# philipturner/metal-flash-attention

Hardware: NVIDIA H100
Metric: giga-FMA-instr/sec forward attn N=4096 D=128 bf16 (higher is better)
Workload: dtype bf16

## Files before the change

### metal-flash-attention_b200/csrc/kernel.cpp

```cpp
#include <cuda_runtime.h>

#include <algorithm>
#include <cmath>
#include <cstring>
#include <map>
#include <mutex>
#include <string>
#include <vector>

#include "internal.h"
#include "kernels/device_state.h"

struct mfa_attention_kernel {
  mfa_attention_kernel_descriptor_t descriptor;
  int type;
  int backend;
  uint32_t threads, smem_bytes, par, trav, head;
  std::string source_name;
  bool windowed;
  mfa_attention_window_t window;
};

namespace mfa {

// ... 245 lines not shown
    if (!precision_pair_valid(mem, reg)) return fail(MFA_ERROR_INVALID_PRECISIONS, "Invalid precisions.");
    if (op != MFA_L && op != MFA_D && !((kd->transpose_state_valid_mask >> op) & 1))
      return fail(MFA_ERROR_INCOMPLETE_DESCRIPTOR,
                  std::string("Transpose state of ") + mfa_operand_name((mfa_operand_t)op) + " was not specified.");
  }

  mfa_attention_kernel *k = new mfa_attention_kernel();
  k->descriptor = *kd;
  k->type = kd->type;
  k->backend = kd->backend;
  const uint32_t D = kd->head_dimension;

  if (k->backend == MFA_BACKEND_TCGEN05) {
    const uint8_t pq = kd->memory_precisions[MFA_Q];
    const uint32_t Dp = (D + 7) / 8 * 8;
    bool ok = (pq == MFA_FP16 || pq == MFA_BF16) && kd->memory_precisions[MFA_K] == pq &&
              kd->memory_precisions[MFA_V] == pq && Dp <= kWgmmaMaxHead;
    bool transposed = false;
    for (int i = 0; i < n; ++i)
      if ((kd->transpose_state_mask >> ops[i]) & 1) transposed = true;
    if (transposed && D % 8 != 0) ok = false;
    if (k->type != MFA_FORWARD && kd->memory_precisions[MFA_dO] != pq &&
        !(pq == MFA_FP16 && kd->memory_precisions[MFA_dO] == MFA_BF16))
      ok = false;
    if (!ok) {
      delete k;
      return fail(MFA_ERROR_UNSUPPORTED,
                  "MFA_BACKEND_TCGEN05 needs FP16/BF16 Q,K,V (row-major for head % 8 != 0; dO of the same "
                  "type, or BF16 with FP16 Q,K,V) and pad8(head) <= the compiled maximum; use MFA_BACKEND_SIMT_FP32 for this "
                  "descriptor.");
    }
    const WgmmaPlan plan = wgmma_plan(k->type, Dp, 1, 1, 1, 1, 0, 1, false, 1);
    k->threads = plan.threads;
    k->smem_bytes = plan.smem_bytes;
    k->par = plan.par;
    k->trav = plan.trav;
    k->head = plan.head;
  } else if (k->backend == MFA_BACKEND_SIMT_FP32) {
    if (D > 512) {
      delete k;
      return fail(MFA_ERROR_UNSUPPORTED, "Head dimension " + std::to_string(D) + " exceeds 512.");
    }
    simt_geometry(k->type, D, &k->threads, &k->smem_bytes, &k->par, &k->trav, &k->head);
  } else {
    delete k;
    return fail(MFA_ERROR_INVALID_ARGUMENT, "Unrecognized backend.");
  }
  if (kd->block_parallelization != k->par || kd->block_traversal != k->trav) {
    std::string msg = "Block dimensions " + std::to_string(kd->block_parallelization) + "x" +
                      std::to_string(kd->block_traversal) + " have no compiled sm_90a kernel (available: " +
                      std::to_string(k->par) + "x" + std::to_string(k->trav) + ").";
    delete k;
    return fail(MFA_ERROR_UNSUPPORTED, msg);
  }
  static const char *typeNames[] = {"forward", "backward_query", "backward_key_value"};
  k->source_name = std::string("attention_") + typeNames[k->type] +
                   (k->backend == MFA_BACKEND_TCGEN05 ? "_tcgen05" : "_simt_fp32") + "<D=" + std::to_string(D) +
                   ">" + (kd->causal ? "_causal" : "");
  k->windowed = false;
  k->window = mfa_attention_window_t{-1, -1};
  *out = k;
  return MFA_SUCCESS;
}

int mfa_attention_kernel_create_windowed(const mfa_attention_kernel_descriptor_t *kd, const mfa_attention_window_t *window,
                                         mfa_attention_kernel_t **out) {
  if (!kd || !out) return fail(MFA_ERROR_INVALID_ARGUMENT, "NULL argument.");
// ... 618 lines not shown
```

### metal-flash-attention_b200/csrc/kernels/attention_params.h

```cpp
#pragma once
#include <cuda_runtime.h>
#include <stdint.h>

namespace mfa {

enum Slot { sQ = 0, sK = 1, sV = 2, sO = 3, sL = 4, sD = 5, sdO = 6, sdV = 7, sdK = 8, sdQ = 9, kSlots = 10 };

enum Prec : uint8_t { FP32 = 0, FP16 = 1, BF16 = 2 };

struct AttentionParams {
  uint32_t R;
  uint32_t C;
  uint32_t D;
  uint32_t batch;
  uint32_t group;
  void *buf[kSlots];
  uint8_t prec[kSlots];
  uint8_t transposed[kSlots];
  float scale;
  float scale_log2;
  uint8_t split_min_blocks;
  uint8_t split_max;
  uint8_t causal;
  int32_t causal_offset;
// ... 52 lines not shown

cudaError_t launch_simt_forward(const AttentionParams &p, const Sequences *seq, const Band *band, cudaStream_t stream);
cudaError_t launch_simt_backward_query(const AttentionParams &p, const Sequences *seq, const Band *band,
                                       cudaStream_t stream);
cudaError_t launch_simt_backward_key_value(const AttentionParams &p, const Sequences *seq, const Band *band,
                                           cudaStream_t stream);
cudaError_t launch_simt_forward_paged(const AttentionParams &p, const PagedKV &pk, const Band *band,
                                      cudaStream_t stream);
void simt_geometry(int type, uint32_t D, uint32_t *threads, uint32_t *smem_bytes, uint32_t *par, uint32_t *trav,
                   uint32_t *head);

constexpr uint32_t kWgmmaMaxHead = 256;
cudaError_t launch_wgmma_forward(const AttentionParams &p, const Sequences *seq, const Band *band, cudaStream_t stream);
cudaError_t launch_wgmma_backward_query(const AttentionParams &p, const Sequences *seq, const Band *band,
                                        cudaStream_t stream);
cudaError_t launch_wgmma_backward_key_value(const AttentionParams &p, const Sequences *seq, const Band *band,
                                            cudaStream_t stream);
cudaError_t launch_wgmma_forward_paged(const AttentionParams &p, const PagedKV &pk, const Band *band,
                                       cudaStream_t stream);
cudaError_t launch_wgmma_forward_split(const AttentionParams &p, const Sequences *seq, const PagedKV *pk,
                                       const Band *band, uint32_t num_splits, uint32_t key_bound, cudaStream_t stream);

struct WgmmaPlan {
  uint32_t threads, smem_bytes;
  uint32_t par, trav, head;
  dim3 grid;
  uint32_t blocks_per_split, splits;
  bool convert_dO_first;
  uint32_t launches;
  uint32_t heads_per_tile;
};
WgmmaPlan wgmma_plan(int type, uint32_t D, uint32_t R, uint32_t C, uint32_t batch, uint32_t group, uint32_t min_blocks,
                     uint32_t max_splits, bool convert_dO, uint32_t sm_count, const Band *band = nullptr);
WgmmaPlan wgmma_plan_sequences(int type, uint32_t D, uint32_t max_row, uint32_t max_column, uint32_t count,
                               uint32_t batch, uint32_t group, bool convert_dO, uint32_t sm_count);
WgmmaPlan wgmma_plan_split(uint32_t D, uint32_t max_row, uint32_t key_bound, uint32_t count, uint32_t batch,
                           uint32_t group, uint32_t min_blocks, uint32_t max_splits, uint32_t num_splits,
                           uint32_t sm_count, const Band *band);

cudaError_t launch_stage_operand(const void *src, void *dst, uint32_t batch, uint32_t seq, uint32_t D, uint32_t Dp,
                                 uint32_t element_bytes, bool transposed, cudaStream_t stream);
cudaError_t launch_unstage_output(const float *src, float *dst, uint32_t batch, uint32_t seq, uint32_t D, uint32_t Dp,
                                  bool transposed, cudaStream_t stream);
cudaError_t launch_unstage_sequences(const float *src, float *dst, uint32_t batch, uint32_t seq, const int32_t *offsets,
                                     uint32_t count, uint32_t limit, uint32_t D, uint32_t Dp, bool transposed,
                                     cudaStream_t stream);
cudaError_t launch_bf16_to_f16(const void *src, void *dst, uint64_t elements, cudaStream_t stream);
const char *last_launch_detail();

}
```

### metal-flash-attention_b200/csrc/kernels/sm90_ptx.cuh

```cuda
#pragma once
#include <cuda_runtime.h>
#include <stdint.h>

namespace mfa {
namespace ptx {

__device__ __forceinline__ uint32_t smem_u32(const void *p) { return static_cast<uint32_t>(__cvta_generic_to_shared(p)); }

__device__ __forceinline__ void mbar_init(uint64_t *bar, uint32_t count) {
  asm volatile("mbarrier.init.shared::cta.b64 [%0], %1;" ::"r"(smem_u32(bar)), "r"(count) : "memory");
}
__device__ __forceinline__ void fence_barrier_init() { asm volatile("fence.mbarrier_init.release.cluster;" ::: "memory"); }
__device__ __forceinline__ void fence_proxy_async_smem() { asm volatile("fence.proxy.async.shared::cta;" ::: "memory"); }

__device__ __forceinline__ void mbar_arrive_expect_tx(uint64_t *bar, uint32_t bytes) {
  asm volatile("mbarrier.arrive.expect_tx.shared::cta.b64 _, [%0], %1;" ::"r"(smem_u32(bar)), "r"(bytes) : "memory");
}
__device__ __forceinline__ void mbar_complete_tx(uint64_t *bar, uint32_t bytes) {
  asm volatile("mbarrier.complete_tx.relaxed.cta.shared::cta.b64 [%0], %1;" ::"r"(smem_u32(bar)), "r"(bytes) : "memory");
}
__device__ __forceinline__ bool mbar_try_wait(uint64_t *bar, uint32_t parity) {
  uint32_t ok;
  asm volatile(
      "{\n"
      ".reg .pred P;\n"
      "mbarrier.try_wait.parity.shared::cta.b64 P, [%1], %2;\n"
      "selp.u32 %0, 1, 0, P;\n"
      "}\n"
      : "=r"(ok)
      : "r"(smem_u32(bar)), "r"(parity)
      : "memory");
  return ok != 0;
}

#ifndef MFA_MBAR_TIMEOUT_CYCLES
#define MFA_MBAR_TIMEOUT_CYCLES (8000000000ll)
#endif
__device__ __forceinline__ void mbar_wait(uint64_t *bar, uint32_t parity) {
  if (mbar_try_wait(bar, parity)) return;
  const long long start = clock64();
  uint32_t spins = 0;
  while (!mbar_try_wait(bar, parity))
    if ((++spins & 0x3ffu) == 0 && clock64() - start > MFA_MBAR_TIMEOUT_CYCLES) __trap();
}

__device__ __forceinline__ void prefetch_tensormap(const void *map) {
  asm volatile("prefetch.tensormap [%0];" ::"l"(reinterpret_cast<uint64_t>(map)) : "memory");
}
__device__ __forceinline__ void tma_load_3d(void *smem_dst, const void *map, uint64_t *bar, int32_t c0, int32_t c1,
                                            int32_t c2) {
  asm volatile(
      "cp.async.bulk.tensor.3d.shared::cluster.global.mbarrier::complete_tx::bytes [%0], [%1, {%3, %4, %5}], [%2];"
      ::"r"(smem_u32(smem_dst)), "l"(reinterpret_cast<uint64_t>(map)), "r"(smem_u32(bar)), "r"(c0), "r"(c1), "r"(c2)
      : "memory");
}

__device__ __forceinline__ uint64_t make_smem_desc_sw128(uint32_t smem_addr, uint32_t lbo_bytes, uint32_t sbo_bytes) {
  uint64_t desc = 0;
  desc |= static_cast<uint64_t>((smem_addr & 0x3FFFFu) >> 4);
  desc |= static_cast<uint64_t>((lbo_bytes >> 4) & 0x3FFFu) << 16;
  desc |= static_cast<uint64_t>((sbo_bytes >> 4) & 0x3FFFu) << 32;
  desc |= static_cast<uint64_t>(1) << 62;
  return desc;
}

__device__ __forceinline__ float ex2_approx(float x) {
  float y;
  asm("ex2.approx.ftz.f32 %0, %1;" : "=f"(y) : "f"(x));
  return y;
}
__device__ __forceinline__ uint32_t pack_bf16x2(float lo, float hi) {
  uint32_t r;
  asm("cvt.rn.bf16x2.f32 %0, %1, %2;" : "=r"(r) : "f"(hi), "f"(lo));
  return r;
}
__device__ __forceinline__ uint32_t pack_f16x2(float lo, float hi) {
  uint32_t r;
  asm("cvt.rn.f16x2.f32 %0, %1, %2;" : "=r"(r) : "f"(hi), "f"(lo));
// ... 6 lines not shown
```

### metal-flash-attention_b200/csrc/kernels/wgmma_attention.cu

```cuda
#include <cuda_fp16.h>
#include <cuda_runtime.h>
#include <math.h>
#include <stdint.h>

#include <type_traits>

#include "attention_params.h"
#include "backward_common.cuh"
#include "device_state.h"
#include "mfa_b200.h"
#include "sm90_ptx.cuh"
#include "tma_host.h"
#include "wgmma.cuh"

namespace mfa {
namespace hop {

using namespace ptx;
using bwd::load_16bit;
using bwd::load_stat;
using bwd::store_stat;

constexpr uint32_t kWG = 128;
constexpr uint32_t kRows = 64;
// ... 266 lines not shown
  }
  const bool empty = kCausal && denom == 0.f;
  const float inv = empty ? 0.f : 1.0f / denom;
  *reinterpret_cast<float4 *>(O + row * D + 4 * quad) = make_float4(acc.x * inv, acc.y * inv, acc.z * inv, acc.w * inv);
  if (quad == 0) store_stat(L, row, l_prec, empty ? INFINITY : lmax + log2f(denom));
}
template <bool kCausal>
__global__ void __launch_bounds__(128) merge_splits(const SplitArgs sp, float *O, void *L, int l_prec, uint64_t rows_total,
                                                    uint32_t D) {
  const uint64_t idx = static_cast<uint64_t>(blockIdx.x) * blockDim.x + threadIdx.x;
  const uint64_t row = idx / (D / 4);
  if (row >= rows_total) return;
  merge_row<kCausal>(sp, O, L, l_prec, rows_total, D, row, static_cast<uint32_t>(idx % (D / 4)));
}

__global__ void __launch_bounds__(128) merge_sequence_splits(const SplitArgs sp, float *O, void *L, int l_prec,
                                                             uint32_t R, uint32_t D, const int32_t *row_offsets) {
  uint32_t q0;
  const uint32_t rows = sequence_rows(row_offsets, blockIdx.z, R, &q0);
  const uint64_t idx = static_cast<uint64_t>(blockIdx.x) * blockDim.x + threadIdx.x, r = idx / (D / 4);
  if (r >= rows) return;
  merge_row<true>(sp, O, L, l_prec, static_cast<uint64_t>(sp.batch) * R, D, static_cast<uint64_t>(blockIdx.y) * R + q0 + r,
                  static_cast<uint32_t>(idx % (D / 4)));
}

template <uint32_t DCH>
struct FwdCfg {
  static constexpr uint32_t kThreads = 2 * kWG, kTileM = 2 * kRows, BN = DCH == 4 ? 64 : 128;
  static constexpr uint32_t kPar = kTileM, kTrav = BN, kQueryBoxRows = kTileM, kKeyBoxRows = BN;
  static constexpr uint32_t kQBytes = DCH * kTileM * 128, kKVBytes = DCH * BN * 128;
  using Smem = SmemLayout<kQBytes, kKVBytes>;
};

enum class KVLayout { kFixed, kPacked, kPaged };

template <uint32_t DCH, uint32_t BN>
__device__ __forceinline__ void load_paged_kv(uint8_t *dst, uint32_t kv_bytes, const CUtensorMap *mapK,
                                              const CUtensorMap *mapV, uint64_t *bar, const PagedKV &pk,
                                              const int32_t *table, uint32_t block, uint32_t box, uint32_t C,
                                              uint32_t kv_head) {
  if (box == BN) {
    const uint32_t row = paged_row(pk, table, block * BN);
#pragma unroll
    for (uint32_t c = 0; c < DCH; ++c) {
      tma_load_3d(dst + c * BN * 128, mapK, bar, c * 64, kv_head, row);
      tma_load_3d(dst + kv_bytes + c * BN * 128, mapV, bar, c * 64, kv_head, row);
    }
    return;
  }
  constexpr uint32_t kMaxBoxes = BN / 16;
  uint32_t rows[kMaxBoxes];
#pragma unroll
  for (uint32_t i = 0; i < kMaxBoxes; ++i) {
    const uint32_t key = block * BN + i * box;
    rows[i] = i * box < BN && key < C ? paged_row(pk, table, key) : 0u;
  }
#pragma unroll
  for (uint32_t i = 0; i < kMaxBoxes; ++i) {
    if (i * box >= BN) break;
#pragma unroll
    for (uint32_t c = 0; c < DCH; ++c) {
      tma_load_3d(dst + c * BN * 128 + i * box * 128, mapK, bar, c * 64, kv_head, rows[i]);
      tma_load_3d(dst + kv_bytes + c * BN * 128 + i * box * 128, mapV, bar, c * 64, kv_head, rows[i]);
    }
  }
}

__device__ __forceinline__ uint2 band_boxes(uint32_t block, uint32_t BN, uint32_t box, int lo, int hi) {
  const int key0 = static_cast<int>(block * BN);
  const int first = max(lo - key0, 0) / static_cast<int>(box);
  const int end = min(hi - key0, static_cast<int>(BN) - 1) / static_cast<int>(box) + 1;
  return make_uint2(static_cast<uint32_t>(first), static_cast<uint32_t>(end));
}
template <uint32_t DCH, uint32_t BN>
__device__ __forceinline__ void load_paged_kv_band(uint8_t *dst, uint32_t kv_bytes, const CUtensorMap *mapK,
                                                   const CUtensorMap *mapV, uint64_t *bar, const PagedKV &pk,
                                                   const int32_t *table, uint32_t block, uint32_t box, int lo, int hi,
                                                   uint32_t kv_head) {
  const uint2 kept = band_boxes(block, BN, box, lo, hi);
  constexpr uint32_t kMaxBoxes = BN / 16;
  uint32_t rows[kMaxBoxes];
#pragma unroll
  for (uint32_t i = 0; i < kMaxBoxes; ++i)
    rows[i] = i >= kept.x && i < kept.y ? paged_row(pk, table, block * BN + i * box) : 0u;
  const uint32_t skipped = BN / box - (kept.y - kept.x);
  if (skipped) mbar_complete_tx(bar, skipped * box * 128 * DCH * 2);
#pragma unroll
  for (uint32_t i = 0; i < kMaxBoxes; ++i) {
    if (i < kept.x || i >= kept.y) continue;
#pragma unroll
    for (uint32_t c = 0; c < DCH; ++c) {
      tma_load_3d(dst + c * BN * 128 + i * box * 128, mapK, bar, c * 64, kv_head, rows[i]);
      tma_load_3d(dst + kv_bytes + c * BN * 128 + i * box * 128, mapV, bar, c * 64, kv_head, rows[i]);
    }
  }
}

template <uint32_t DCH, bool kBF16, bool kCausal, KVLayout kLayout, bool kBand = false, bool kSplit = false>
__device__ __forceinline__ void forward_body(const CUtensorMap &mapQ, const CUtensorMap &mapK, const CUtensorMap &mapV,
                                             float *__restrict__ O, void *__restrict__ L, uint32_t R, uint32_t C,
                                             uint32_t D, float scale_log2, int l_prec, const SplitArgs &sp, int delta,
                                             uint32_t group, const Sequences &seq, const PagedKV &pk,
                                             const Band &band = Band{}, uint32_t hpt = 1) {
  constexpr bool kVarlen = kLayout != KVLayout::kFixed;
  static_assert(!kSplit || kVarlen, "the fixed-length forward splits through blockIdx.z");
  using Cfg = FwdCfg<DCH>;
  constexpr uint32_t NO = DCH * 64, BN = Cfg::BN;
  extern __shared__ uint8_t smem_raw[];
  const Ring<typename Cfg::Smem> ring(smem_raw);
  const uint32_t tid = threadIdx.x, wg = tid / kWG, t = tid % kWG;
  const uint32_t tile = kSplit ? blockIdx.x / sp.splits : blockIdx.x;
  const uint32_t tile_rows = kSplit ? Cfg::kTileM / hpt : Cfg::kTileM;
  const uint32_t head = blockIdx.y, row_base = tile * tile_rows;
  const uint32_t kv_head = (kSplit ? head * hpt : head) / group;
  SequenceSpan span{0, R, 0, C};
  uint32_t kb0, per_split;
  if constexpr (kVarlen) {
    span = kLayout == KVLayout::kPaged ? paged_span(pk, blockIdx.z) : sequence_span(seq, blockIdx.z);
    if (row_base >= span.R) return;
    delta = static_cast<int>(span.C) - static_cast<int>(span.R);
    kb0 = 0;
    per_split = (span.C + BN - 1) / BN;
  } else {
    kb0 = blockIdx.z * sp.blocks_per_split;
    per_split = sp.blocks_per_split;
  }
  uint32_t blocks;
// ... 2 lines not shown
                             : make_int2(0, static_cast<int>(key_blocks<BN, kCausal>(row_base, tile_rows, span.R,
                                                                                     span.C, delta, 0, per_split)));
    const uint32_t n = static_cast<uint32_t>(max(range.y - range.x, 0));
    blocks = band_split(range, blockIdx.x % sp.splits, (n + sp.splits - 1) / sp.splits, &kb0);
  } else if constexpr (kBand) {
    blocks = band_split(band_key_blocks<BN>(row_base, Cfg::kTileM, span.R, span.C, delta, band),
                        kVarlen ? 0u : blockIdx.z, per_split, &kb0);
  } else {
    blocks = key_blocks<BN, kCausal>(row_base, Cfg::kTileM, span.R, span.C, delta, kb0, per_split);
  }
  const int64_t band_last = static_cast<int64_t>(min(row_base + tile_rows, span.R)) - 1;
  const int band_lo = kBand ? static_cast<int>(max(static_cast<int64_t>(row_base) + delta - band.left, int64_t(-1))) : 0;
  const int band_hi = kBand ? static_cast<int>(min(band_last + delta + band.right, static_cast<int64_t>(span.C))) : 0;

  const int32_t *table = kLayout == KVLayout::kPaged ? pk.page_table + static_cast<size_t>(blockIdx.z) * pk.page_stride
                                                     : nullptr;
  const uint32_t box = kLayout == KVLayout::kPaged ? min(1u << pk.page_shift, BN) : BN;
  auto load_kv = [&](uint32_t j, uint8_t *dst, uint64_t *bar) {
    if constexpr (kLayout == KVLayout::kPaged && kBand) {
      load_paged_kv_band<DCH, BN>(dst, Cfg::kKVBytes, &mapK, &mapV, bar, pk, table, kb0 + j, box, band_lo,
                                  min(band_hi, static_cast<int>(span.C) - 1), kv_head);
    } else if constexpr (kLayout == KVLayout::kPaged) {
      load_paged_kv<DCH, BN>(dst, Cfg::kKVBytes, &mapK, &mapV, bar, pk, table, kb0 + j, box, span.C, kv_head);
    } else {
      load_tile<DCH, BN>(dst, &mapK, bar, span.k0 + (kb0 + j) * BN, kv_head);
      load_tile<DCH, BN>(dst + Cfg::kKVBytes, &mapV, bar, span.k0 + (kb0 + j) * BN, kv_head);
    }
  };
  if (tid == 0) {
    prefetch_tensormap(&mapQ);
    prefetch_tensormap(&mapK);
    prefetch_tensormap(&mapV);
  }
  ring.init();
  ring.start(
      [&](uint8_t *dst, uint64_t *bar) {
        load_tile<DCH, Cfg::kTileM>(dst, &mapQ, bar, span.q0 + row_base, kSplit ? head * hpt : head);
        if (kSplit && hpt * tile_rows < Cfg::kTileM) mbar_complete_tx(bar, (Cfg::kTileM - hpt * tile_rows) * 128 * DCH);
      },
      blocks, load_kv);

  const uint32_t sQ = smem_u32(ring.base);
  float o[NO / 2];
  zero(o);
  float m0 = -INFINITY, m1 = -INFINITY, l0 = 0.f, l1 = 0.f;
  const uint32_t trow0 = wg * kRows + frag_row(t);
  const int qrow0 = static_cast<int>(row_base + trow0 % tile_rows);
  const int qrow1 = static_cast<int>(row_base + (trow0 + 8) % tile_rows);
  ring.wait_resident();
  for (uint32_t j = 0; j < blocks; ++j) {
    ring.wait(j);
    if constexpr (kLayout == KVLayout::kPaged && kBand) {
      const uint2 kept = band_boxes(kb0 + j, BN, box, band_lo, min(band_hi, static_cast<int>(span.C) - 1));
      const uint32_t first = kept.x * box, end = min(kept.y * box, span.C - (kb0 + j) * BN);
      if (first > 0 || end < BN) {
        zero_row_range<DCH, BN, Cfg::kThreads>(ring.stage(j), 0, first);
        zero_row_range<DCH, BN, Cfg::kThreads>(ring.stage(j), end, BN);
        zero_row_range<DCH, BN, Cfg::kThreads>(ring.stage(j) + Cfg::kKVBytes, 0, first);
        zero_row_range<DCH, BN, Cfg::kThreads>(ring.stage(j) + Cfg::kKVBytes, end, BN);
        fence_proxy_async_smem();
        __syncthreads();
      }
    } else if (kVarlen && ((kBand || kSplit ? kb0 : 0) + j + 1) * BN > span.C) {
      const uint32_t kb = (kBand || kSplit ? kb0 : 0) + j;
      zero_rows<DCH, BN, Cfg::kThreads>(ring.stage(j), span.C - kb * BN);
      zero_rows<DCH, BN, Cfg::kThreads>(ring.stage(j) + Cfg::kKVBytes, span.C - kb * BN);
      fence_proxy_async_smem();
      __syncthreads();
    }
    const uint32_t sK = smem_u32(ring.stage(j)), sV = sK + Cfg::kKVBytes;
    float sc[BN / 2];
    zero(sc);
    wgmma_fence();
    mma_ss<DCH, BN, kBF16, Cfg::kTileM>(sc, sQ, wg * kRows, sK);
    wgmma_commit();
    wgmma_wait<0>();
    fence_regs(sc);

    if ((kb0 + j + 1) * BN > span.C) mask_past_edge(sc, (kb0 + j) * BN, span.C);
    if constexpr (kSplit) {
      const int key0 = static_cast<int>((kb0 + j) * BN);
      const int64_t lower = kBand ? static_cast<int64_t>(delta) - band.left : -(int64_t(1) << 40);
      const int64_t upper = static_cast<int64_t>(delta) + (kBand ? band.right : 0);
      if ((kBand || kCausal) && crosses_band(key0, key0 + static_cast<int>(BN) - 1, static_cast<int>(row_base),
                                             static_cast<int>(row_base + tile_rows) - 1, lower, upper))
        mask_rows_outside_band(sc, qrow0, qrow1, key0, lower, upper);
    } else if constexpr (kBand) {
      const int key0 = static_cast<int>((kb0 + j) * BN), row = static_cast<int>(row_base + wg * kRows + frag_row(t));
      const int64_t lower = static_cast<int64_t>(delta) - band.left, upper = static_cast<int64_t>(delta) + band.right;
      if (crosses_band(key0, key0 + static_cast<int>(BN) - 1, static_cast<int>(row_base),
                       static_cast<int>(row_base + Cfg::kTileM) - 1, lower, upper))
        mask_outside_band<false>(sc, row, key0, lower, upper);
    } else if constexpr (kCausal) {
      const int key0 = static_cast<int>((kb0 + j) * BN);
      if (crosses_diagonal(key0 + static_cast<int>(BN) - 1, static_cast<int>(row_base), delta))
        mask_past_diagonal<false>(sc, static_cast<int>(row_base + wg * kRows + frag_row(t)), key0, delta);
    }
    float r0 = -INFINITY, r1 = -INFINITY;
#pragma unroll
    for (uint32_t i = 0; i < BN / 8; ++i) {
      r0 = fmaxf(r0, fmaxf(sc[4 * i], sc[4 * i + 1]));
      r1 = fmaxf(r1, fmaxf(sc[4 * i + 2], sc[4 * i + 3]));
    }
    r0 = fmaxf(r0, __shfl_xor_sync(0xffffffffu, r0, 1));
    r0 = fmaxf(r0, __shfl_xor_sync(0xffffffffu, r0, 2));
    r1 = fmaxf(r1, __shfl_xor_sync(0xffffffffu, r1, 1));
    r1 = fmaxf(r1, __shfl_xor_sync(0xffffffffu, r1, 2));
    const float mn0 = fmaxf(m0, r0 * scale_log2), mn1 = fmaxf(m1, r1 * scale_log2);
    const float ref0 = kCausal && mn0 == -INFINITY ? 0.f : mn0, ref1 = kCausal && mn1 == -INFINITY ? 0.f : mn1;
    const float a0 = ex2_approx(m0 - ref0), a1 = ex2_approx(m1 - ref1);
    m0 = mn0;
    m1 = mn1;
    l0 *= a0;
    l1 *= a1;
#pragma unroll
    for (uint32_t i = 0; i < NO / 8; ++i) {
      o[4 * i] *= a0;
      o[4 * i + 1] *= a0;
      o[4 * i + 2] *= a1;
      o[4 * i + 3] *= a1;
    }
#pragma unroll
    for (uint32_t i = 0; i < BN / 8; ++i) {
      sc[4 * i] = ex2_approx(fmaf(sc[4 * i], scale_log2, -ref0));
      sc[4 * i + 1] = ex2_approx(fmaf(sc[4 * i + 1], scale_log2, -ref0));
      sc[4 * i + 2] = ex2_approx(fmaf(sc[4 * i + 2], scale_log2, -ref1));
      sc[4 * i + 3] = ex2_approx(fmaf(sc[4 * i + 3], scale_log2, -ref1));
      l0 += sc[4 * i] + sc[4 * i + 1];
      l1 += sc[4 * i + 2] + sc[4 * i + 3];
    }
    wgmma_fence();
#pragma unroll
    for (uint32_t kk = 0; kk < BN / 16; ++kk) {
      uint32_t a[4];
      a_frag<kBF16>(sc, kk, a);
      Wgmma<NO, kBF16>::rs(o, a, desc_mnmajor<BN>(sV, kk, 0), 1);
      if constexpr (DCH == 1) {
        wgmma_commit();
        wgmma_wait<0>();
      }
    }
    wgmma_commit();
    wgmma_wait<0>();
    fence_regs(o);
    ring.release_and_refill(j, blocks, load_kv);
  }

  l0 += __shfl_xor_sync(0xffffffffu, l0, 1);
  l0 += __shfl_xor_sync(0xffffffffu, l0, 2);
  l1 += __shfl_xor_sync(0xffffffffu, l1, 1);
  l1 += __shfl_xor_sync(0xffffffffu, l1, 2);
  if constexpr (kSplit) {
    const uint32_t split = blockIdx.x % sp.splits;
#pragma unroll
    for (uint32_t h = 0; h < 2; ++h) {
      const uint32_t trow = trow0 + 8 * h, r = row_base + trow % tile_rows, qh = head * hpt + trow / tile_rows;
      if (trow >= hpt * tile_rows || r >= span.R) continue;
      const float l = h ? l1 : l0, mrow = h ? m1 : m0, inv = l == 0.f ? 0.f : 1.0f / l;
      const size_t row = (sp.splits == 1 ? static_cast<size_t>(qh) : static_cast<size_t>(split) * sp.batch + qh) * R +
                         span.q0 + r;
      float *out = (sp.splits == 1 ? O : sp.O_part) + row * D;
#pragma unroll
      for (int i = 0; i < NO / 8; ++i) {
        const uint32_t col = 8 * i + 2 * (t % 4);
        if (col < D)
          *reinterpret_cast<float2 *>(out + col) = make_float2(o[4 * i + 2 * h] * inv, o[4 * i + 2 * h + 1] * inv);
      }
      if (t % 4 == 0)
        store_stat(sp.splits == 1 ? L : sp.L_part, row, sp.splits == 1 ? l_prec : FP32,
                   l == 0.f ? (sp.splits == 1 ? INFINITY : -INFINITY) : mrow + log2f(l));
    }
    return;
  }
  const uint32_t row0 = row_base + wg * kRows;
  const size_t slice = static_cast<size_t>(blockIdx.z) * sp.batch + head;
  float *Oout = sp.splits == 1 ? O + (static_cast<size_t>(head) * R + span.q0) * D : sp.O_part + slice * R * D;
  const bool empty0 = (kCausal || kVarlen) && l0 == 0.f, empty1 = (kCausal || kVarlen) && l1 == 0.f;
  store_acc(o, Oout, row0, span.R, 0, D, empty0 ? 0.f : 1.0f / l0, empty1 ? 0.f : 1.0f / l1);
// ... 554 lines not shown
  if ((e = make_tensor_map_16bit(&m->Q, p.buf[sQ], p.R, p.D, p.batch, Cfg::kQueryBoxRows)) != cudaSuccess) return e;
  if (with_dO &&
      (e = make_tensor_map_16bit(&m->dO, p.buf[sdO], p.R, p.D, p.batch, Cfg::kQueryBoxRows)) != cudaSuccess)
    return e;
  const uint32_t kv_heads = p.batch / p.group;
  if ((e = make_tensor_map_16bit(&m->K, p.buf[sK], p.C, p.D, kv_heads, Cfg::kKeyBoxRows)) != cudaSuccess) return e;
  return make_tensor_map_16bit(&m->V, p.buf[sV], p.C, p.D, kv_heads, Cfg::kKeyBoxRows);
}

template <uint32_t DCH, bool kBF16, bool kCausal>
cudaError_t launch_forward(const AttentionParams &p, const WgmmaPlan &plan, const Sequences *seq, const Band *band,
                           cudaStream_t stream) {
  using Cfg = FwdCfg<DCH>;
  constexpr uint32_t kSmemBytes = Cfg::Smem::kSmemBytes;
  auto kernel = attention_forward_wgmma<DCH, kBF16, kCausal>;
  TensorMaps m;
  cudaError_t e;
  if (seq && band) {
    auto packed = band_forward_packed_wgmma<DCH, kBF16>;
    if ((e = prepare(packed, kSmemBytes)) != cudaSuccess || (e = make_maps<Cfg>(p, false, &m)) != cudaSuccess) return e;
    packed<<<plan.grid, Cfg::kThreads, kSmemBytes, stream>>>(m.Q, m.K, m.V, static_cast<float *>(p.buf[sO]),
                                                             p.buf[sL], p.R, p.C, p.D, p.scale_log2, p.prec[sL],
                                                             p.group, *seq, *band);
    return cudaGetLastError();
  }
  if (seq) {
    auto packed = packed_forward_wgmma<DCH, kBF16, kCausal>;
    if ((e = prepare(packed, kSmemBytes)) != cudaSuccess || (e = make_maps<Cfg>(p, false, &m)) != cudaSuccess) return e;
    packed<<<plan.grid, Cfg::kThreads, kSmemBytes, stream>>>(m.Q, m.K, m.V, static_cast<float *>(p.buf[sO]),
                                                             p.buf[sL], p.R, p.C, p.D, p.scale_log2, p.prec[sL],
                                                             p.group, *seq);
    return cudaGetLastError();
  }
  if ((e = (band ? prepare(band_forward_wgmma<DCH, kBF16>, kSmemBytes) : prepare(kernel, kSmemBytes))) != cudaSuccess ||
      (e = make_maps<Cfg>(p, false, &m)) != cudaSuccess)
    return e;
  SplitArgs sp{plan.blocks_per_split, plan.splits, p.batch, nullptr, nullptr};
  const uint64_t rows_total = static_cast<uint64_t>(p.batch) * p.R;
  if (plan.splits > 1) {
    void *ws = nullptr;
    const size_t o_elems = plan.splits * rows_total * p.D;
    if ((e = workspace_for(current_device(), stream, (o_elems + plan.splits * rows_total) * sizeof(float), &ws)) !=
        cudaSuccess)
      return e;
    sp.O_part = static_cast<float *>(ws);
    sp.L_part = sp.O_part + o_elems;
  }
  if (band)
    band_forward_wgmma<DCH, kBF16><<<plan.grid, Cfg::kThreads, kSmemBytes, stream>>>(
        m.Q, m.K, m.V, static_cast<float *>(p.buf[sO]), p.buf[sL], p.R, p.C, p.D, p.scale_log2, p.prec[sL], sp,
        p.causal_offset, p.group, *band);
  else
    kernel<<<plan.grid, Cfg::kThreads, kSmemBytes, stream>>>(m.Q, m.K, m.V, static_cast<float *>(p.buf[sO]), p.buf[sL],
                                                             p.R, p.C, p.D, p.scale_log2, p.prec[sL], sp,
                                                             p.causal_offset, p.group);
  if ((e = cudaGetLastError()) != cudaSuccess || plan.splits == 1) return e;
  const uint64_t threads = rows_total * (p.D / 4);
  auto merge = band ? merge_splits<true> : merge_splits<kCausal>;
  merge<<<static_cast<uint32_t>((threads + 127) / 128), 128, 0, stream>>>(sp, static_cast<float *>(p.buf[sO]), p.buf[sL],
                                                                          p.prec[sL], rows_total, p.D);
  return cudaGetLastError();
}

template <uint32_t DCH, bool kBF16, bool kCausal>
cudaError_t launch_forward_paged(const AttentionParams &p, const WgmmaPlan &plan, const PagedKV &pk, const Band *band,
                                 cudaStream_t stream) {
  using Cfg = FwdCfg<DCH>;
  constexpr uint32_t kSmemBytes = Cfg::Smem::kSmemBytes;
  auto kernel = paged_forward_wgmma<DCH, kBF16, kCausal>;
  const uint32_t box = min(1u << pk.page_shift, Cfg::BN);
  TensorMaps m;
  cudaError_t e;
  if ((e = (band ? prepare(band_forward_paged_wgmma<DCH, kBF16>, kSmemBytes) : prepare(kernel, kSmemBytes))) !=
          cudaSuccess ||
      (e = make_tensor_map_16bit(&m.Q, p.buf[sQ], p.R, p.D, p.batch, Cfg::kQueryBoxRows)) != cudaSuccess ||
      (e = make_tensor_map_page_pool(&m.K, p.buf[sK], p.C, pk.kv_heads, p.D, box)) != cudaSuccess ||
      (e = make_tensor_map_page_pool(&m.V, p.buf[sV], p.C, pk.kv_heads, p.D, box)) != cudaSuccess)
    return e;
  if (band)
    band_forward_paged_wgmma<DCH, kBF16><<<plan.grid, Cfg::kThreads, kSmemBytes, stream>>>(
        m.Q, m.K, m.V, static_cast<float *>(p.buf[sO]), p.buf[sL], p.R, p.D, p.scale_log2, p.prec[sL], p.group, pk,
        *band);
  else
    kernel<<<plan.grid, Cfg::kThreads, kSmemBytes, stream>>>(m.Q, m.K, m.V, static_cast<float *>(p.buf[sO]), p.buf[sL],
                                                             p.R, p.D, p.scale_log2, p.prec[sL], p.group, pk);
  return cudaGetLastError();
}

// ... 93 lines not shown
  float *scratch = nullptr;
  if (plan.splits > 1) {
    void *ws = nullptr;
    if ((e = workspace_for(current_device(), stream, plan.splits * outputs * elems * sizeof(float), &ws)) != cudaSuccess)
      return e;
    scratch = static_cast<float *>(ws);
    a.split_stride = outputs * elems;
    a.*out0 = scratch;
    if (out1) a.*out1 = scratch + elems;
  }
  kernel<<<plan.grid, Cfg::kThreads, kSmemBytes, stream>>>(m.Q, m.dO, m.K, m.V, a, extra...);
  if ((e = cudaGetLastError()) != cudaSuccess || plan.splits == 1) return e;
  const size_t quads = elems / 4;
  sum_splits<<<dim3(static_cast<uint32_t>((quads + 255) / 256), outputs), 256, 0, stream>>>(
      reinterpret_cast<const float4 *>(scratch), reinterpret_cast<float4 *>(dst0), reinterpret_cast<float4 *>(dst1), quads,
      a.split_stride / 4, plan.splits);
  return cudaGetLastError();
}

template <class F>
static cudaError_t dispatch(const AttentionParams &p, bool convert_dO, F f) {
  return with_chunks(p.D, [&](auto dch) {
    auto types = [&](auto causal) {
      if (convert_dO) return f(dch, std::false_type(), std::true_type(), causal);
      if (p.prec[sQ] == BF16) return f(dch, std::true_type(), std::false_type(), causal);
      return f(dch, std::false_type(), std::false_type(), causal);
    };
    return p.causal ? types(std::true_type()) : types(std::false_type());
  });
}

}

WgmmaPlan wgmma_plan(int type, uint32_t D, uint32_t R, uint32_t C, uint32_t batch, uint32_t group, uint32_t min_blocks,
                     uint32_t max_splits, bool convert_dO, uint32_t sm_count, const Band *band) {
  WgmmaPlan p{};
  p.heads_per_tile = 1;
  auto geometry = [&](auto cfg) {
    using Cfg = decltype(cfg);
    p.threads = Cfg::kThreads;
    p.smem_bytes = Cfg::Smem::kSmemBytes;
    p.par = Cfg::kPar;
    p.trav = Cfg::kTrav;
  };
  hop::with_chunks(D, [&](auto dch) {
    constexpr uint32_t DCH = decltype(dch)::value;
    if (type == MFA_FORWARD)
      geometry(hop::FwdCfg<DCH>());
    else if (type == MFA_BACKWARD_QUERY)
      geometry(hop::QCfg<DCH>());
    else
      geometry(hop::KVCfg<DCH>());
  });
  const uint32_t padded = (D + 7) / 8 * 8, columns = hop::chunks(D) * 64;
  p.head = columns < padded ? columns : padded;

  const bool key_value = type == MFA_BACKWARD_KEY_VALUE;
  const uint32_t tiles = ((key_value ? C : R) + p.par - 1) / p.par;
  uint32_t total = ((key_value ? R : C) + p.trav - 1) / p.trav;
  if (band) {
    const uint64_t width = (static_cast<uint64_t>(p.par) + band->left + band->right + p.trav - 1) / p.trav + 1;
    if (width < total) total = static_cast<uint32_t>(width);
  }
  const uint32_t heads = key_value ? batch / group : batch;
  if (type == MFA_FORWARD) {
    p.splits = hop::choose_splits(tiles * heads, total, sm_count, min_blocks, max_splits);
// ... 155 lines not shown
```

Baseline: 297,900.

## Add software-pipelined non-causal forward path with separate K/V stage barriers

For D=128 non-causal fixed-layout forward, a new path overlaps the QK^T wgmma of block j with the PV wgmma of block j-1, so tensor-core work hides the softmax latency. K and V get separate 3-stage full barriers, and warps release stages through a shared-memory atomic counter that triggers the refill TMA. The smem size differs for this path and is reported to the host. The risks are higher register pressure from holding both score and output accumulators live, and more complex synchronization.

```diff
diff --git a/metal-flash-attention_b200/csrc/kernel.cpp b/metal-flash-attention_b200/csrc/kernel.cpp
--- a/metal-flash-attention_b200/csrc/kernel.cpp
+++ b/metal-flash-attention_b200/csrc/kernel.cpp
@@ -301,7 +301,7 @@
     }
     const WgmmaPlan plan = wgmma_plan(k->type, Dp, 1, 1, 1, 1, 0, 1, false, 1);
     k->threads = plan.threads;
-    k->smem_bytes = plan.smem_bytes;
+    k->smem_bytes = k->type == MFA_FORWARD ? wgmma_forward_smem_bytes(Dp, kd->causal) : plan.smem_bytes;
     k->par = plan.par;
     k->trav = plan.trav;
     k->head = plan.head;
diff --git a/metal-flash-attention_b200/csrc/kernels/attention_params.h b/metal-flash-attention_b200/csrc/kernels/attention_params.h
--- a/metal-flash-attention_b200/csrc/kernels/attention_params.h
+++ b/metal-flash-attention_b200/csrc/kernels/attention_params.h
@@ -108,6 +108,7 @@
 };
 WgmmaPlan wgmma_plan(int type, uint32_t D, uint32_t R, uint32_t C, uint32_t batch, uint32_t group, uint32_t min_blocks,
                      uint32_t max_splits, bool convert_dO, uint32_t sm_count, const Band *band = nullptr);
+uint32_t wgmma_forward_smem_bytes(uint32_t D, bool causal);
 WgmmaPlan wgmma_plan_sequences(int type, uint32_t D, uint32_t max_row, uint32_t max_column, uint32_t count,
                                uint32_t batch, uint32_t group, bool convert_dO, uint32_t sm_count);
 WgmmaPlan wgmma_plan_split(uint32_t D, uint32_t max_row, uint32_t key_bound, uint32_t count, uint32_t batch,
diff --git a/metal-flash-attention_b200/csrc/kernels/sm90_ptx.cuh b/metal-flash-attention_b200/csrc/kernels/sm90_ptx.cuh
--- a/metal-flash-attention_b200/csrc/kernels/sm90_ptx.cuh
+++ b/metal-flash-attention_b200/csrc/kernels/sm90_ptx.cuh
@@ -44,6 +44,12 @@
     if ((++spins & 0x3ffu) == 0 && clock64() - start > MFA_MBAR_TIMEOUT_CYCLES) __trap();
 }
 
+__device__ __forceinline__ uint32_t atomic_add_acq_rel(uint32_t *p, uint32_t v) {
+  uint32_t old;
+  asm volatile("atom.acq_rel.cta.shared::cta.add.u32 %0, [%1], %2;" : "=r"(old) : "r"(smem_u32(p)), "r"(v) : "memory");
+  return old;
+}
+
 __device__ __forceinline__ void prefetch_tensormap(const void *map) {
   asm volatile("prefetch.tensormap [%0];" ::"l"(reinterpret_cast<uint64_t>(map)) : "memory");
 }
diff --git a/metal-flash-attention_b200/csrc/kernels/wgmma_attention.cu b/metal-flash-attention_b200/csrc/kernels/wgmma_attention.cu
--- a/metal-flash-attention_b200/csrc/kernels/wgmma_attention.cu
+++ b/metal-flash-attention_b200/csrc/kernels/wgmma_attention.cu
@@ -322,6 +322,60 @@
   using Smem = SmemLayout<kQBytes, kKVBytes>;
 };
 
+template <uint32_t DCH, bool kCausal>
+constexpr bool kPipelinedForward = DCH == 2 && !kCausal;
+
+template <uint32_t DCH>
+struct PipeSmem {
+  static constexpr uint32_t kStages = 3;
+  static constexpr uint32_t kKOffset = FwdCfg<DCH>::kQBytes, kVOffset = kKOffset + kStages * FwdCfg<DCH>::kKVBytes;
+  static constexpr uint32_t kBarOffset = kVOffset + kStages * FwdCfg<DCH>::kKVBytes, kBars = 1 + 2 * kStages + kStages;
+  static constexpr uint32_t kSmemBytes = 1024 + kBarOffset + kBars * 8;
+};
+
+template <int NR>
+__device__ __forceinline__ void scale_rows(float (&o)[NR], float a0, float a1) {
+#pragma unroll
+  for (int i = 0; i < NR / 4; ++i) {
+    o[4 * i] *= a0;
+    o[4 * i + 1] *= a0;
+    o[4 * i + 2] *= a1;
+    o[4 * i + 3] *= a1;
+  }
+}
+
+template <bool kCausal, int NR>
+__device__ __forceinline__ void softmax_block(float (&sc)[NR], float scale_log2, float &m0, float &m1, float &l0,
+                                              float &l1, float &a0, float &a1) {
+  float r0 = -INFINITY, r1 = -INFINITY;
+#pragma unroll
+  for (int i = 0; i < NR / 4; ++i) {
+    r0 = fmaxf(r0, fmaxf(sc[4 * i], sc[4 * i + 1]));
+    r1 = fmaxf(r1, fmaxf(sc[4 * i + 2], sc[4 * i + 3]));
+  }
+  r0 = fmaxf(r0, __shfl_xor_sync(0xffffffffu, r0, 1));
+  r0 = fmaxf(r0, __shfl_xor_sync(0xffffffffu, r0, 2));
+  r1 = fmaxf(r1, __shfl_xor_sync(0xffffffffu, r1, 1));
+  r1 = fmaxf(r1, __shfl_xor_sync(0xffffffffu, r1, 2));
+  const float mn0 = fmaxf(m0, r0 * scale_log2), mn1 = fmaxf(m1, r1 * scale_log2);
+  const float ref0 = kCausal && mn0 == -INFINITY ? 0.f : mn0, ref1 = kCausal && mn1 == -INFINITY ? 0.f : mn1;
+  a0 = ex2_approx(m0 - ref0);
+  a1 = ex2_approx(m1 - ref1);
+  m0 = mn0;
+  m1 = mn1;
+  l0 *= a0;
+  l1 *= a1;
+#pragma unroll
+  for (int i = 0; i < NR / 4; ++i) {
+    sc[4 * i] = ex2_approx(fmaf(sc[4 * i], scale_log2, -ref0));
+    sc[4 * i + 1] = ex2_approx(fmaf(sc[4 * i + 1], scale_log2, -ref0));
+    sc[4 * i + 2] = ex2_approx(fmaf(sc[4 * i + 2], scale_log2, -ref1));
+    sc[4 * i + 3] = ex2_approx(fmaf(sc[4 * i + 3], scale_log2, -ref1));
+    l0 += sc[4 * i] + sc[4 * i + 1];
+    l1 += sc[4 * i + 2] + sc[4 * i + 3];
+  }
+}
+
 enum class KVLayout { kFixed, kPacked, kPaged };
 
 template <uint32_t DCH, uint32_t BN>
@@ -383,6 +437,106 @@
       tma_load_3d(dst + c * BN * 128 + i * box * 128, mapK, bar, c * 64, kv_head, rows[i]);
       tma_load_3d(dst + kv_bytes + c * BN * 128 + i * box * 128, mapV, bar, c * 64, kv_head, rows[i]);
     }
+  }
+}
+
+template <uint32_t DCH, bool kBF16>
+__device__ __forceinline__ void forward_pipelined(const CUtensorMap &mapQ, const CUtensorMap &mapK,
+                                                  const CUtensorMap &mapV, uint8_t *smem_raw, uint32_t row_base,
+                                                  uint32_t head, uint32_t kv_head, uint32_t kb0, uint32_t blocks,
+                                                  uint32_t C, float scale_log2, float (&o)[DCH * 32], float &m0,
+                                                  float &m1, float &l0, float &l1) {
+  using Cfg = FwdCfg<DCH>;
+  constexpr uint32_t NO = DCH * 64, BN = Cfg::BN;
+  const uint32_t tid = threadIdx.x, wg = tid / kWG;
+  using Pipe = PipeSmem<DCH>;
+  constexpr uint32_t S = Pipe::kStages;
+  uint8_t *base = align1024(smem_raw);
+  uint64_t *const qbar = reinterpret_cast<uint64_t *>(base + Pipe::kBarOffset);
+  uint64_t *const fullK = qbar + 1, *const fullV = fullK + S;
+  uint32_t *const released = reinterpret_cast<uint32_t *>(fullV + S);
+  auto load_block = [&](uint32_t n) {
+    const uint32_t s = n % S, key = (kb0 + n) * BN;
+    mbar_arrive_expect_tx(&fullK[s], Cfg::kKVBytes);
+    load_tile<DCH, BN>(base + Pipe::kKOffset + s * Cfg::kKVBytes, &mapK, &fullK[s], key, kv_head);
+    mbar_arrive_expect_tx(&fullV[s], Cfg::kKVBytes);
+    load_tile<DCH, BN>(base + Pipe::kVOffset + s * Cfg::kKVBytes, &mapV, &fullV[s], key, kv_head);
+  };
+  if (tid == 0) {
+    mbar_init(qbar, 1);
+    for (uint32_t s = 0; s < S; ++s) {
+      mbar_init(&fullK[s], 1);
+      mbar_init(&fullV[s], 1);
+      released[s] = 0;
+    }
+    fence_barrier_init();
+  }
+  __syncthreads();
+  if (tid == 0) {
+    mbar_arrive_expect_tx(qbar, Cfg::kQBytes);
+    load_tile<DCH, Cfg::kTileM>(base, &mapQ, qbar, row_base, head);
+    for (uint32_t n = 0; n < S && n < blocks; ++n) load_block(n);
+  }
+  auto release = [&](uint32_t j) {
+    if (j + S < blocks && tid % 32 == 0 && atomic_add_acq_rel(&released[j % S], 1u) % 8 == 7) load_block(j + S);
+  };
+  const uint32_t sQ = smem_u32(base), sK = sQ + Pipe::kKOffset, sV = sQ + Pipe::kVOffset;
+  auto mask_block = [&](float(&sc)[BN / 2], uint32_t j) {
+    if ((kb0 + j + 1) * BN > C) mask_past_edge(sc, (kb0 + j) * BN, C);
+  };
+  auto issue_s = [&](float(&sc)[BN / 2], uint32_t j) {
+    mbar_wait(&fullK[j % S], (j / S) & 1);
+    mma_ss<DCH, BN, kBF16, Cfg::kTileM>(sc, sQ, wg * kRows, sK + (j % S) * Cfg::kKVBytes);
+    wgmma_commit();
+  };
+  auto issue_pv = [&](const uint32_t(&p)[BN / 4], uint32_t j) {
+    mbar_wait(&fullV[j % S], (j / S) & 1);
+#pragma unroll
+    for (uint32_t kk = 0; kk < BN / 16; ++kk) {
+      const uint32_t a[4] = {p[4 * kk], p[4 * kk + 1], p[4 * kk + 2], p[4 * kk + 3]};
+      Wgmma<NO, kBF16>::rs(o, a, desc_mnmajor<BN>(sV + (j % S) * Cfg::kKVBytes, kk, 0), 1);
+    }
+    wgmma_commit();
+  };
+  auto pack = [&](const float(&sc)[BN / 2], uint32_t(&p)[BN / 4]) {
+#pragma unroll
+    for (uint32_t i = 0; i < BN / 4; ++i) p[i] = pack2<kBF16>(sc[2 * i], sc[2 * i + 1]);
+  };
+  mbar_wait(qbar, 0);
+  if (blocks > 0) {
+    uint32_t p[BN / 4];
+    {
+      float sc[BN / 2];
+      wgmma_fence();
+      issue_s(sc, 0);
+      wgmma_wait<0>();
+      fence_regs(sc);
+      mask_block(sc, 0);
+      float a0, a1;
+      softmax_block<false>(sc, scale_log2, m0, m1, l0, l1, a0, a1);
+      pack(sc, p);
+    }
+    for (uint32_t j = 1; j < blocks; ++j) {
+      float sc[BN / 2];
+      wgmma_fence();
+      issue_s(sc, j);
+      issue_pv(p, j - 1);
+      wgmma_wait<1>();
+      fence_regs(sc);
+      mask_block(sc, j);
+      float a0, a1;
+      softmax_block<false>(sc, scale_log2, m0, m1, l0, l1, a0, a1);
+      wgmma_wait<0>();
+      fence_regs(o);
+      fence_regs(sc);
+      release(j - 1);
+      scale_rows(o, a0, a1);
+      pack(sc, p);
+    }
+    wgmma_fence();
+    issue_pv(p, blocks - 1);
+    wgmma_wait<0>();
+    fence_regs(o);
   }
 }
 
@@ -451,13 +605,16 @@
     prefetch_tensormap(&mapK);
     prefetch_tensormap(&mapV);
   }
-  ring.init();
-  ring.start(
-      [&](uint8_t *dst, uint64_t *bar) {
-        load_tile<DCH, Cfg::kTileM>(dst, &mapQ, bar, span.q0 + row_base, kSplit ? head * hpt : head);
-        if (kSplit && hpt * tile_rows < Cfg::kTileM) mbar_complete_tx(bar, (Cfg::kTileM - hpt * tile_rows) * 128 * DCH);
-      },
-      blocks, load_kv);
+  constexpr bool kPipelined = kLayout == KVLayout::kFixed && !kBand && kPipelinedForward<DCH, kCausal>;
+  if constexpr (!kPipelined) {
+    ring.init();
+    ring.start(
+        [&](uint8_t *dst, uint64_t *bar) {
+          load_tile<DCH, Cfg::kTileM>(dst, &mapQ, bar, span.q0 + row_base, kSplit ? head * hpt : head);
+          if (kSplit && hpt * tile_rows < Cfg::kTileM) mbar_complete_tx(bar, (Cfg::kTileM - hpt * tile_rows) * 128 * DCH);
+        },
+        blocks, load_kv);
+  }
 
   const uint32_t sQ = smem_u32(ring.base);
   float o[NO / 2];
@@ -466,103 +623,108 @@
   const uint32_t trow0 = wg * kRows + frag_row(t);
   const int qrow0 = static_cast<int>(row_base + trow0 % tile_rows);
   const int qrow1 = static_cast<int>(row_base + (trow0 + 8) % tile_rows);
-  ring.wait_resident();
-  for (uint32_t j = 0; j < blocks; ++j) {
-    ring.wait(j);
-    if constexpr (kLayout == KVLayout::kPaged && kBand) {
-      const uint2 kept = band_boxes(kb0 + j, BN, box, band_lo, min(band_hi, static_cast<int>(span.C) - 1));
-      const uint32_t first = kept.x * box, end = min(kept.y * box, span.C - (kb0 + j) * BN);
-      if (first > 0 || end < BN) {
-        zero_row_range<DCH, BN, Cfg::kThreads>(ring.stage(j), 0, first);
-        zero_row_range<DCH, BN, Cfg::kThreads>(ring.stage(j), end, BN);
-        zero_row_range<DCH, BN, Cfg::kThreads>(ring.stage(j) + Cfg::kKVBytes, 0, first);
-        zero_row_range<DCH, BN, Cfg::kThreads>(ring.stage(j) + Cfg::kKVBytes, end, BN);
+  if constexpr (kPipelined) {
+    forward_pipelined<DCH, kBF16>(mapQ, mapK, mapV, smem_raw, row_base, head, kv_head, kb0, blocks, span.C, scale_log2,
+                                  o, m0, m1, l0, l1);
+  } else {
+    ring.wait_resident();
+    for (uint32_t j = 0; j < blocks; ++j) {
+      ring.wait(j);
+      if constexpr (kLayout == KVLayout::kPaged && kBand) {
+        const uint2 kept = band_boxes(kb0 + j, BN, box, band_lo, min(band_hi, static_cast<int>(span.C) - 1));
+        const uint32_t first = kept.x * box, end = min(kept.y * box, span.C - (kb0 + j) * BN);
+        if (first > 0 || end < BN) {
+          zero_row_range<DCH, BN, Cfg::kThreads>(ring.stage(j), 0, first);
+          zero_row_range<DCH, BN, Cfg::kThreads>(ring.stage(j), end, BN);
+          zero_row_range<DCH, BN, Cfg::kThreads>(ring.stage(j) + Cfg::kKVBytes, 0, first);
+          zero_row_range<DCH, BN, Cfg::kThreads>(ring.stage(j) + Cfg::kKVBytes, end, BN);
+          fence_proxy_async_smem();
+          __syncthreads();
+        }
+      } else if (kVarlen && ((kBand || kSplit ? kb0 : 0) + j + 1) * BN > span.C) {
+        const uint32_t kb = (kBand || kSplit ? kb0 : 0) + j;
+        zero_rows<DCH, BN, Cfg::kThreads>(ring.stage(j), span.C - kb * BN);
+        zero_rows<DCH, BN, Cfg::kThreads>(ring.stage(j) + Cfg::kKVBytes, span.C - kb * BN);
         fence_proxy_async_smem();
         __syncthreads();
       }
-    } else if (kVarlen && ((kBand || kSplit ? kb0 : 0) + j + 1) * BN > span.C) {
-      const uint32_t kb = (kBand || kSplit ? kb0 : 0) + j;
-      zero_rows<DCH, BN, Cfg::kThreads>(ring.stage(j), span.C - kb * BN);
-      zero_rows<DCH, BN, Cfg::kThreads>(ring.stage(j) + Cfg::kKVBytes, span.C - kb * BN);
-      fence_proxy_async_smem();
-      __syncthreads();
-    }
-    const uint32_t sK = smem_u32(ring.stage(j)), sV = sK + Cfg::kKVBytes;
-    float sc[BN / 2];
-    zero(sc);
-    wgmma_fence();
-    mma_ss<DCH, BN, kBF16, Cfg::kTileM>(sc, sQ, wg * kRows, sK);
-    wgmma_commit();
-    wgmma_wait<0>();
-    fence_regs(sc);
-
-    if ((kb0 + j + 1) * BN > span.C) mask_past_edge(sc, (kb0 + j) * BN, span.C);
-    if constexpr (kSplit) {
-      const int key0 = static_cast<int>((kb0 + j) * BN);
-      const int64_t lower = kBand ? static_cast<int64_t>(delta) - band.left : -(int64_t(1) << 40);
-      const int64_t upper = static_cast<int64_t>(delta) + (kBand ? band.right : 0);
-      if ((kBand || kCausal) && crosses_band(key0, key0 + static_cast<int>(BN) - 1, static_cast<int>(row_base),
-                                             static_cast<int>(row_base + tile_rows) - 1, lower, upper))
-        mask_rows_outside_band(sc, qrow0, qrow1, key0, lower, upper);
-    } else if constexpr (kBand) {
-      const int key0 = static_cast<int>((kb0 + j) * BN), row = static_cast<int>(row_base + wg * kRows + frag_row(t));
-      const int64_t lower = static_cast<int64_t>(delta) - band.left, upper = static_cast<int64_t>(delta) + band.right;
-      if (crosses_band(key0, key0 + static_cast<int>(BN) - 1, static_cast<int>(row_base),
-                       static_cast<int>(row_base + Cfg::kTileM) - 1, lower, upper))
-        mask_outside_band<false>(sc, row, key0, lower, upper);
-    } else if constexpr (kCausal) {
-      const int key0 = static_cast<int>((kb0 + j) * BN);
-      if (crosses_diagonal(key0 + static_cast<int>(BN) - 1, static_cast<int>(row_base), delta))
-        mask_past_diagonal<false>(sc, static_cast<int>(row_base + wg * kRows + frag_row(t)), key0, delta);
-    }
-    float r0 = -INFINITY, r1 = -INFINITY;
-#pragma unroll
-    for (uint32_t i = 0; i < BN / 8; ++i) {
-      r0 = fmaxf(r0, fmaxf(sc[4 * i], sc[4 * i + 1]));
-      r1 = fmaxf(r1, fmaxf(sc[4 * i + 2], sc[4 * i + 3]));
-    }
-    r0 = fmaxf(r0, __shfl_xor_sync(0xffffffffu, r0, 1));
-    r0 = fmaxf(r0, __shfl_xor_sync(0xffffffffu, r0, 2));
-    r1 = fmaxf(r1, __shfl_xor_sync(0xffffffffu, r1, 1));
-    r1 = fmaxf(r1, __shfl_xor_sync(0xffffffffu, r1, 2));
-    const float mn0 = fmaxf(m0, r0 * scale_log2), mn1 = fmaxf(m1, r1 * scale_log2);
-    const float ref0 = kCausal && mn0 == -INFINITY ? 0.f : mn0, ref1 = kCausal && mn1 == -INFINITY ? 0.f : mn1;
-    const float a0 = ex2_approx(m0 - ref0), a1 = ex2_approx(m1 - ref1);
-    m0 = mn0;
-    m1 = mn1;
-    l0 *= a0;
-    l1 *= a1;
-#pragma unroll
-    for (uint32_t i = 0; i < NO / 8; ++i) {
-      o[4 * i] *= a0;
-      o[4 * i + 1] *= a0;
-      o[4 * i + 2] *= a1;
-      o[4 * i + 3] *= a1;
-    }
-#pragma unroll
-    for (uint32_t i = 0; i < BN / 8; ++i) {
-      sc[4 * i] = ex2_approx(fmaf(sc[4 * i], scale_log2, -ref0));
-      sc[4 * i + 1] = ex2_approx(fmaf(sc[4 * i + 1], scale_log2, -ref0));
-      sc[4 * i + 2] = ex2_approx(fmaf(sc[4 * i + 2], scale_log2, -ref1));
-      sc[4 * i + 3] = ex2_approx(fmaf(sc[4 * i + 3], scale_log2, -ref1));
-      l0 += sc[4 * i] + sc[4 * i + 1];
-      l1 += sc[4 * i + 2] + sc[4 * i + 3];
-    }
-    wgmma_fence();
-#pragma unroll
-    for (uint32_t kk = 0; kk < BN / 16; ++kk) {
-      uint32_t a[4];
-      a_frag<kBF16>(sc, kk, a);
-      Wgmma<NO, kBF16>::rs(o, a, desc_mnmajor<BN>(sV, kk, 0), 1);
-      if constexpr (DCH == 1) {
-        wgmma_commit();
-        wgmma_wait<0>();
+      const uint32_t sK = smem_u32(ring.stage(j)), sV = sK + Cfg::kKVBytes;
+      float sc[BN / 2];
+      zero(sc);
+      wgmma_fence();
+      mma_ss<DCH, BN, kBF16, Cfg::kTileM>(sc, sQ, wg * kRows, sK);
+      wgmma_commit();
+      wgmma_wait<0>();
+      fence_regs(sc);
+
+      if ((kb0 + j + 1) * BN > span.C) mask_past_edge(sc, (kb0 + j) * BN, span.C);
+      if constexpr (kSplit) {
+        const int key0 = static_cast<int>((kb0 + j) * BN);
+        const int64_t lower = kBand ? static_cast<int64_t>(delta) - band.left : -(int64_t(1) << 40);
+        const int64_t upper = static_cast<int64_t>(delta) + (kBand ? band.right : 0);
+        if ((kBand || kCausal) && crosses_band(key0, key0 + static_cast<int>(BN) - 1, static_cast<int>(row_base),
+                                               static_cast<int>(row_base + tile_rows) - 1, lower, upper))
+          mask_rows_outside_band(sc, qrow0, qrow1, key0, lower, upper);
+      } else if constexpr (kBand) {
+        const int key0 = static_cast<int>((kb0 + j) * BN), row = static_cast<int>(row_base + wg * kRows + frag_row(t));
+        const int64_t lower = static_cast<int64_t>(delta) - band.left, upper = static_cast<int64_t>(delta) + band.right;
+        if (crosses_band(key0, key0 + static_cast<int>(BN) - 1, static_cast<int>(row_base),
+                         static_cast<int>(row_base + Cfg::kTileM) - 1, lower, upper))
+          mask_outside_band<false>(sc, row, key0, lower, upper);
+      } else if constexpr (kCausal) {
+        const int key0 = static_cast<int>((kb0 + j) * BN);
+        if (crosses_diagonal(key0 + static_cast<int>(BN) - 1, static_cast<int>(row_base), delta))
+          mask_past_diagonal<false>(sc, static_cast<int>(row_base + wg * kRows + frag_row(t)), key0, delta);
       }
-    }
-    wgmma_commit();
-    wgmma_wait<0>();
-    fence_regs(o);
-    ring.release_and_refill(j, blocks, load_kv);
+      float r0 = -INFINITY, r1 = -INFINITY;
+#pragma unroll
+      for (uint32_t i = 0; i < BN / 8; ++i) {
+        r0 = fmaxf(r0, fmaxf(sc[4 * i], sc[4 * i + 1]));
+        r1 = fmaxf(r1, fmaxf(sc[4 * i + 2], sc[4 * i + 3]));
+      }
+      r0 = fmaxf(r0, __shfl_xor_sync(0xffffffffu, r0, 1));
+      r0 = fmaxf(r0, __shfl_xor_sync(0xffffffffu, r0, 2));
+      r1 = fmaxf(r1, __shfl_xor_sync(0xffffffffu, r1, 1));
+      r1 = fmaxf(r1, __shfl_xor_sync(0xffffffffu, r1, 2));
+      const float mn0 = fmaxf(m0, r0 * scale_log2), mn1 = fmaxf(m1, r1 * scale_log2);
+      const float ref0 = kCausal && mn0 == -INFINITY ? 0.f : mn0, ref1 = kCausal && mn1 == -INFINITY ? 0.f : mn1;
+      const float a0 = ex2_approx(m0 - ref0), a1 = ex2_approx(m1 - ref1);
+      m0 = mn0;
+      m1 = mn1;
+      l0 *= a0;
+      l1 *= a1;
+#pragma unroll
+      for (uint32_t i = 0; i < NO / 8; ++i) {
+        o[4 * i] *= a0;
+        o[4 * i + 1] *= a0;
+        o[4 * i + 2] *= a1;
+        o[4 * i + 3] *= a1;
+      }
+#pragma unroll
+      for (uint32_t i = 0; i < BN / 8; ++i) {
+        sc[4 * i] = ex2_approx(fmaf(sc[4 * i], scale_log2, -ref0));
+        sc[4 * i + 1] = ex2_approx(fmaf(sc[4 * i + 1], scale_log2, -ref0));
+        sc[4 * i + 2] = ex2_approx(fmaf(sc[4 * i + 2], scale_log2, -ref1));
+        sc[4 * i + 3] = ex2_approx(fmaf(sc[4 * i + 3], scale_log2, -ref1));
+        l0 += sc[4 * i] + sc[4 * i + 1];
+        l1 += sc[4 * i + 2] + sc[4 * i + 3];
+      }
+      wgmma_fence();
+#pragma unroll
+      for (uint32_t kk = 0; kk < BN / 16; ++kk) {
+        uint32_t a[4];
+        a_frag<kBF16>(sc, kk, a);
+        Wgmma<NO, kBF16>::rs(o, a, desc_mnmajor<BN>(sV, kk, 0), 1);
+        if constexpr (DCH == 1) {
+          wgmma_commit();
+          wgmma_wait<0>();
+        }
+      }
+      wgmma_commit();
+      wgmma_wait<0>();
+      fence_regs(o);
+      ring.release_and_refill(j, blocks, load_kv);
+    }
   }
 
   l0 += __shfl_xor_sync(0xffffffffu, l0, 1);
@@ -1183,7 +1345,9 @@
                                                              p.group, *seq);
     return cudaGetLastError();
   }
-  if ((e = (band ? prepare(band_forward_wgmma<DCH, kBF16>, kSmemBytes) : prepare(kernel, kSmemBytes))) != cudaSuccess ||
+  constexpr uint32_t kFixedSmemBytes = kPipelinedForward<DCH, kCausal> ? PipeSmem<DCH>::kSmemBytes : kSmemBytes;
+  if ((e = (band ? prepare(band_forward_wgmma<DCH, kBF16>, kSmemBytes) : prepare(kernel, kFixedSmemBytes))) !=
+          cudaSuccess ||
       (e = make_maps<Cfg>(p, false, &m)) != cudaSuccess)
     return e;
   SplitArgs sp{plan.blocks_per_split, plan.splits, p.batch, nullptr, nullptr};
@@ -1202,9 +1366,9 @@
         m.Q, m.K, m.V, static_cast<float *>(p.buf[sO]), p.buf[sL], p.R, p.C, p.D, p.scale_log2, p.prec[sL], sp,
         p.causal_offset, p.group, *band);
   else
-    kernel<<<plan.grid, Cfg::kThreads, kSmemBytes, stream>>>(m.Q, m.K, m.V, static_cast<float *>(p.buf[sO]), p.buf[sL],
-                                                             p.R, p.C, p.D, p.scale_log2, p.prec[sL], sp,
-                                                             p.causal_offset, p.group);
+    kernel<<<plan.grid, Cfg::kThreads, kFixedSmemBytes, stream>>>(m.Q, m.K, m.V, static_cast<float *>(p.buf[sO]),
+                                                                  p.buf[sL], p.R, p.C, p.D, p.scale_log2, p.prec[sL],
+                                                                  sp, p.causal_offset, p.group);
   if ((e = cudaGetLastError()) != cudaSuccess || plan.splits == 1) return e;
   const uint64_t threads = rows_total * (p.D / 4);
   auto merge = band ? merge_splits<true> : merge_splits<kCausal>;
@@ -1364,6 +1528,14 @@
 
 }
 
+uint32_t wgmma_forward_smem_bytes(uint32_t D, bool causal) {
+  return hop::with_chunks(D, [&](auto dch) {
+    constexpr uint32_t DCH = decltype(dch)::value;
+    return hop::kPipelinedForward<DCH, false> && !causal ? hop::PipeSmem<DCH>::kSmemBytes
+                                                         : hop::FwdCfg<DCH>::Smem::kSmemBytes;
+  });
+}
+
 WgmmaPlan wgmma_plan(int type, uint32_t D, uint32_t R, uint32_t C, uint32_t batch, uint32_t group, uint32_t min_blocks,
                      uint32_t max_splits, bool convert_dO, uint32_t sm_count, const Band *band) {
   WgmmaPlan p{};
```

Result: faster. 306,000 (median of 6 runs) (+2.7%).
